# bitmagier/q-learning

Hardware: AMD Instinct MI355X
Metric: env-steps/sec + grad-updates/sec, Breakout 84×84×4, 1/2/4/8 MI355X (higher is better)
Workload: dtype fp32; 1 GPU; C3: 8192 Breakout envs per GPU, replay 1000000 per GPU in HBM (prefilled), Nature-DQN (3 conv + 2 dense) in fp32, B=1024, update every 128 env-steps per GPU (replay ratio 8 samples/env-step), epsilon-greedy acting; envs_per_gpu=8192, batch=1024, replay_capacity=1000000, update_after_actions=128, parallelism=single, rccl_world=1, global_batch_per_update=1024, env_dtype=fp32 physics, u8 frames, qnet_dtype=fp32 (exact-fp32 MFMA v_mfma_f32_16x16x4_f32)

## Files before the change

### q-learning_amd/csrc/qnet32_kernels.h

```cpp
#pragma once
#include <hip/hip_runtime.h>

#include <cstdint>
#include <type_traits>

#include "qlx_internal.h"

namespace qlx {
namespace q32 {

typedef float f32x4 __attribute__((ext_vector_type(4)));

constexpr int BK = 32;
constexpr int kListSlots = 8;
constexpr int kCntStride = 16;

__host__ __device__ constexpr int kmaj_pad(int rows, int r) { return rows + ((r - rows % 64) % 64 + 64) % 64; }
__host__ __device__ constexpr int kmaj_pitch(int rows) {
  return kmaj_pad(rows, 48) < kmaj_pad(rows, 16) ? kmaj_pad(rows, 48) : kmaj_pad(rows, 16);
}
static_assert(kmaj_pitch(32) == 48 && kmaj_pitch(64) == 80 && kmaj_pitch(128) == 144, "KMAJ pitches");

template <int ROWS, bool KMAJ>
struct Opnd {
// ... 409 lines not shown
#pragma unroll
    for (int i = 0; i < N; ++i) {
      const int idx = tid + i * T;
      int r = 0, k = 0;
      if (O::F4 % T == 0 || idx < O::F4) O::coord(idx, r, k);
      vo[i] = lane_off(r, k);
      kk[i] = k;
    }
  }
  __device__ void load(uint32_t soff, int kvalid, Regs& rg) const {
    if (!KMASK || kvalid >= BK) {
#pragma unroll
      for (int i = 0; i < N; ++i)
        if (O::F4 % T == 0 || tid + i * T < O::F4) rg[i] = buf_ld4(rs, vo[i], soff);
    } else {
#pragma unroll
      for (int i = 0; i < N; ++i)
        if (O::F4 % T == 0 || tid + i * T < O::F4) rg[i] = buf_ld4(rs, kk[i] < kvalid ? vo[i] : kOob, soff);
    }
  }
  __device__ void store(float* t, const Regs& rg) const {
#pragma unroll
    for (int i = 0; i < N; ++i) {
      const int idx = tid + i * T;
      if (O::F4 % T == 0 || idx < O::F4) {
        int r, k;
        O::coord(idx, r, k);
        O::put(t, r, k, rg[i]);
      }
    }
  }
};

template <class SA, class SB, uint32_t DA, uint32_t DB, bool KMASK = false>
struct PairStreams {
  SA a;
  SB b;
  int kmax;
  struct Regs {
    typename SA::Regs a;
    typename SB::Regs b;
  };
  __device__ void load(int s, Regs& x) const {
    const int kv = kmax - s * BK;
    a.load((uint32_t)s * DA, kv, x.a);
    b.load((uint32_t)s * DB, kv, x.b);
  }
  __device__ void store(float* as, float* bs, const Regs& x) const {
    a.store(as, x.a);
    b.store(bs, x.b);
  }
};

template <int T, bool PADS = true, int SHIFT = 0, uint32_t MASK = 0xFFFFFFFFu, uint32_t MUL = 1u>
struct TableK4Stream {
  static_assert(T == 256, "table gather stream: four waves");
  using O = Opnd<64, true>;
  static constexpr int N = 2;
  static constexpr uint32_t PAST = SHIFT == 0 && MASK == 0xFFFFFFFFu ? kOob : MASK * MUL;
  using Regs = f32x4[N];
  Rsrc rs;
  uint32_t vo;
  int tid, g, k0;
  const uint32_t* tbl;
  static constexpr int IMG = Opnd<64, true>::FLOATS, PITCH = Opnd<64, true>::PITCH;
  static_assert(PITCH == 80, "table stream: 16 pad columns per k-row");
  __host__ __device__ static int slot(int r) { return PADS ? (r >> 9) * IMG + ((r >> 4) & 31) * PITCH + 64 + (r & 15) : 4 * IMG + r; }
  __device__ void init(const void* base, uint32_t bytes, int tid_, uint32_t row_off) {
    rs = buf_rsrc(base, bytes);
    tid = tid_;
    g = (tid & 63) >> 4;
    k0 = q32_uniform(tid >> 6) * 4;
    vo = row_off;
  }
  __device__ void load(int kbase, Regs& rg) const {
#pragma unroll
    for (int i = 0; i < N; ++i) rg[i] = buf_ld4(rs, vo + ((tbl[slot(kbase + k0 + 16 * i + g)] >> SHIFT) & MASK) * MUL, 0u);
  }
  __device__ void store(float* t, const Regs& rg) const {
#pragma unroll
    for (int i = 0; i < N; ++i) O::put(t, (tid & 15) * 4, k0 + 16 * i + g, rg[i]);
  }
};

template <class P, class = void>
struct ExtraLdsOf : std::integral_constant<size_t, 0> {};
template <class P>
struct ExtraLdsOf<P, std::void_t<decltype(P::EXTRA_LDS)>> : std::integral_constant<size_t, P::EXTRA_LDS> {};

template <class S, class = void>
struct HasPrepare : std::false_type {};
template <class S>
struct HasPrepare<S, std::void_t<decltype(std::declval<S&>().prepare((float*)nullptr, 0))>> : std::true_type {};

template <class P>
constexpr size_t gemm_lds_bytes() {
  return (size_t)KSplitOf<P>::value * 2 *
             (size_t)(Opnd<P::BM, P::A_KMAJ>::FLOATS + Opnd<P::BN, P::B_KMAJ>::FLOATS) * sizeof(float) +
         ExtraLdsOf<P>::value;
}

template <class P, class = void>
struct HasStreams : std::false_type {};
template <class P>
struct HasStreams<P, std::void_t<typename P::Streams>> : std::true_type {};

template <class P>
__device__ __forceinline__ void gemm_body_s(const P& p, int lb, float* lds) {
  constexpr int MF = 16;
  using OA = Opnd<P::BM, P::A_KMAJ>;
  using OB = Opnd<P::BN, P::B_KMAJ>;
  using Acc = f32x4;
  constexpr int TM = P::BM / (P::WM * MF), TN = P::BN / (P::WN * MF);
  static_assert(TM >= 1 && TN >= 1 && TM * P::WM * MF == P::BM && TN * P::WN * MF == P::BN, "tile shape");
  constexpr int G = KSplitOf<P>::value, Q = KSeqOf<P>::value;
  static_assert((G == 1 && Q <= 2) || (Q == 1 && !P::BIAS), "K split: two sequential chains, or wave groups without bias");
  static_assert(G == 1 || TM * TN * 4 * P::WM * P::WN * 64 <= 2 * (OA::FLOATS + OB::FLOATS), "K-split hand-off fits a group's LDS");
  constexpr int T = P::WM * P::WN * 64;
  constexpr int GROUP_LDS = 2 * (OA::FLOATS + OB::FLOATS);
  using St = typename P::Streams;
  using Regs = typename St::Regs;
  const int kg = G > 1 ? __builtin_amdgcn_readfirstlane((int)(threadIdx.x >> 6) / (P::WM * P::WN)) : 0;
  const int tid = threadIdx.x - kg * T, lane = tid & 63;
  const int wave = __builtin_amdgcn_readfirstlane(tid >> 6);
  const int wm = wave % P::WM, wn = wave / P::WM;
  int tm, tn, z;
  p.decode(lb, tm, tn, z);
  const int row0 = tm * P::BM, col0 = tn * P::BN;
  if constexpr (HasActive<P>::value) {
    if (!p.active(z, row0)) return;
  }
  const int ns = p.nslabs(z) / G, s_base = kg * ns;
  const int s_half = Q > 1 ? ns / 2 : -1;
  St st = p.streams(z, row0, col0, tid);
  lds += kg * GROUP_LDS;
  float* As0 = lds;
  float* As1 = lds + OA::FLOATS;
  float* Bs0 = lds + 2 * OA::FLOATS;
  float* Bs1 = Bs0 + OB::FLOATS;
  if constexpr (HasPrepare<St>::value) {
    st.prepare(lds, ns);
    __syncthreads();
  }
  Regs x0, x1;
  Acc acc[TM][TN];
#pragma unroll
  for (int i = 0; i < TM; ++i)
#pragma unroll
    for (int j = 0; j < TN; ++j) acc[i][j] = zero4();
  Acc first[Q > 1 ? TM : 1][Q > 1 ? TN : 1];
  float bsum[TN];
#pragma unroll
  for (int j = 0; j < TN; ++j) bsum[j] = 0.0f;
  const bool do_bias = P::BIAS && tm == 0 && wm == 0;
  auto slab_loop = [&](auto bias_tag) {
    constexpr bool DB = decltype(bias_tag)::value;
    auto compute = [&](int s) {
      const float* a = (s & 1) ? As1 : As0;
      const float* b = (s & 1) ? Bs1 : Bs0;
      if constexpr (Q > 1) {
        if (s == s_half) {
#pragma unroll
          for (int i = 0; i < TM; ++i)
#pragma unroll
            for (int j = 0; j < TN; ++j) {
              first[i][j] = acc[i][j];
// ... 552 lines not shown
    const int m = M;
    st.a.init(dz4, (uint32_t)M * 512u * 4u, tid,
              [row0, m](int r, int k) { return row0 + r < m ? (uint32_t)((row0 + r) * 512 + k) * 4u : kOob; });
    st.b.init(w3, 3136u * 512u * 4u, tid, [col0](int r, int k) { return (uint32_t)((col0 + r) * 512 + k) * 4u; });
    st.kmax = 512;
    return st;
  }
};
using PFc1DgradS = PFc1DgradT<32, 64, 2, 2>;

template <int BM_, int BN_, int WM_, int WN_>
struct PFc1WgradT {
  static constexpr int BM = BM_, BN = BN_, WM = WM_, WN = WN_;
  static constexpr int MINW = 6;
  static constexpr bool A_KMAJ = true, B_KMAJ = true, BIAS = true;
  Grid g;
  const float* a3;
  const float* dz4;
  float* dw3;
  float* db3;
  int B;
  __host__ __device__ void decode(int lb, int& tm, int& tn, int& z) const { g.decode(lb, tm, tn, z); }
  __host__ __device__ int nslabs(int) const { return (B + BK - 1) / BK; }
  __device__ void epi(int, int row, int col, f32x4 v) const {
#pragma unroll
    for (int r = 0; r < 4; ++r)
      if (row + r < 3136) dw3[(size_t)(row + r) * 512 + col] = v[r];
  }
  __device__ void epi_bias(int, int col, float v) const { db3[col] = v; }
  static constexpr int T = WM_ * WN_ * 64;
  using SA = AffineStream<BM_, true, T, true>;
  using SB = AffineStream<BN_, true, T, true>;
  using Streams = PairStreams<SA, SB, BK * 3136u * 4u, BK * 512u * 4u, true>;
  __device__ Streams streams(int, int row0, int col0, int tid) const {
    Streams st;
    st.a.init(a3, (uint32_t)B * 3136u * 4u, tid, [row0](int r, int k) { return (uint32_t)(k * 3136 + row0 + r) * 4u; });
    st.b.init(dz4, (uint32_t)B * 512u * 4u, tid, [col0](int r, int k) { return (uint32_t)(k * 512 + col0 + r) * 4u; });
    st.kmax = B;
    return st;
  }
};
using PFc1WgradS = PFc1WgradT<64, 32, 2, 2>;

__host__ __device__ inline int px3_order(int z) { return z < 5 ? z + 2 : (z == 5 ? 1 : (z == 6 ? 7 : (z == 7 ? 0 : 8))); }
__host__ __device__ inline int px2_order(int z) { return z < 8 ? z + 1 : (z == 8 ? 0 : 9); }

template <int BM_, int BN_, int WM_, int WN_>
struct PConv3DgradPx {
  static constexpr int BM = BM_, BN = BN_, WM = WM_, WN = WN_;
  static constexpr bool LOAD_FENCE = false;
  static constexpr bool A_KMAJ = false, B_KMAJ = false, BIAS = false, RAW_ORDER = true;
  Grid g;
  const float* dz3;
  const float* w2;
  const float* a2;
  float* dz2;
  int B;
  float* pbg = nullptr;
  const uint8_t* bg2 = nullptr;
  int bg2_ld = 0;
  __host__ __device__ void decode(int lb, int& tm, int& tn, int& z) const { g.decode(lb, tm, tn, z); }
  struct Px {
    int ih, iw, kh0, kw0, nkw, ntap;
  };
  struct Pre {
    f32x4 m;
    uint32_t bg;
  };
  __host__ __device__ static Px px(int z) {
    Px q;
    q.ih = px3_order(z / 9);
    q.iw = px3_order(z % 9);
    q.kh0 = q.ih > 6 ? q.ih - 6 : 0;
    q.kw0 = q.iw > 6 ? q.iw - 6 : 0;
    const int kh1 = q.ih < 2 ? q.ih : 2, kw1 = q.iw < 2 ? q.iw : 2;
    q.nkw = kw1 - q.kw0 + 1;
    q.ntap = (kh1 - q.kh0 + 1) * q.nkw;
    return q;
  }
  __host__ __device__ int nslabs(int z) const { return 2 * px(z).ntap; }
  __device__ void epi(int z, int row, int col, f32x4 v) const { epi_post(z, row, col, v, epi_pre(z, row, col)); }
  __device__ Pre epi_pre(int z, int row, int col) const {
    const Px q = px(z);
    Pre pr;
#pragma unroll
    for (int r = 0; r < 4; ++r) pr.m[r] = a2[((size_t)((row + r < B ? row + r : 0) * 9 + q.ih) * 9 + q.iw) * 64 + col];
    pr.bg = pbg ? *reinterpret_cast<const uint32_t*>(bg2 + (size_t)(q.ih * 9 + q.iw) * bg2_ld + row) : 0u;
    return pr;
  }
  __device__ void epi_post(int z, int row, int col, f32x4 v, const Pre& pr) const {
    const Px q = px(z);
    float d[4], e[4];
#pragma unroll
    for (int r = 0; r < 4; ++r) {
      d[r] = row + r < B && pr.m[r] > 0.0f ? v[r] : 0.0f;
      e[r] = ((pr.bg >> (8 * r)) & 0xFFu) != 0u ? d[r] : 0.0f;
      if (row + r < B) dz2[((size_t)((row + r) * 9 + q.ih) * 9 + q.iw) * 64 + col] = d[r];
    }
    if (pbg) {
      const float s = pb_sum16(e);
      if ((row & 15) == 0 && row < B) pbg[((size_t)(row >> 4) * 81 + q.ih * 9 + q.iw) * 64 + col] = s;
    }
  }
  static constexpr int T = WM_ * WN_ * 64;
  struct Streams {
    AffineStream<BM_, false, T> a;
    AffineStream<BN_, false, T> b;
    struct Regs {
      typename AffineStream<BM_, false, T>::Regs a;
      typename AffineStream<BN_, false, T>::Regs b;
    };
    int z0;
    __device__ void load(int s, Regs& x) const {
      const Px q = px(z0);
      const int t = s >> 1, kh = q.kh0 + t / q.nkw, kw = q.kw0 + t % q.nkw, h = (s & 1) * 32;
      a.load((uint32_t)(((q.ih - kh) * 7 + q.iw - kw) * 64 + h) * 4u, 0, x.a);
      b.load((uint32_t)((kh * 3 + kw) * 4096 + h) * 4u, 0, x.b);
    }
    __device__ void store(float* as, float* bs, const Regs& x) const {
      a.store(as, x.a);
      b.store(bs, x.b);
    }
  };
  __device__ Streams streams(int z, int row0, int col0, int tid) const {
    Streams st;
    st.z0 = z;
    const int nb = B;
    st.a.init(dz3, (uint32_t)B * 3136u * 4u, tid,
              [row0, nb](int r, int k) { return row0 + r < nb ? (uint32_t)((row0 + r) * 3136 + k) * 4u : kOob; });
    st.b.init(w2, 9u * 4096u * 4u, tid, [col0](int r, int k) { return (uint32_t)((col0 + r) * 64 + k) * 4u; });
    return st;
  }
};

template <int BM_, int BN_, int WM_, int WN_>
struct PConv2DgradPx {
  static constexpr int BM = BM_, BN = BN_, WM = WM_, WN = WN_;
  static constexpr bool LOAD_FENCE = false;
  static constexpr bool A_KMAJ = false, B_KMAJ = false, BIAS = false, RAW_ORDER = true;
  Grid g;
  const float* dz2;
  const float* w1;
  const float* a1;
  float* dz1;
  int B;
  float* pb = nullptr;
  const uint8_t* need = nullptr;
  int need_ld = 0;
  __host__ __device__ void decode(int lb, int& tm, int& tn, int& z) const { g.decode(lb, tm, tn, z); }
  struct Px {
    int i, j, th0, tw0, ntw, ntap;
  };
  struct Pre {
    f32x4 m;
    uint32_t nb;
  };
  __host__ __device__ static Px px(int z) {
    Px q;
    q.i = px2_order(z / 10);
    q.j = px2_order(z % 10);
    q.th0 = q.i == 9 ? 1 : 0;
    q.tw0 = q.j == 9 ? 1 : 0;
    const int th1 = q.i == 0 ? 0 : 1, tw1 = q.j == 0 ? 0 : 1;
    q.ntw = tw1 - q.tw0 + 1;
    q.ntap = (th1 - q.th0 + 1) * q.ntw;
    return q;
  }
  __host__ __device__ int nslabs(int z) const { return 2 * px(z).ntap; }
  __device__ void epi(int z, int row, int col, f32x4 v) const { epi_post(z, row, col, v, epi_pre(z, row, col)); }
  __device__ Pre epi_pre(int z, int row, int col) const {
    const Px q = px(z);
    const int cls = col >> 5, ih = 2 * q.i + (cls >> 1), iw = 2 * q.j + (cls & 1);
    Pre pr;
#pragma unroll
    for (int r = 0; r < 4; ++r) pr.m[r] = a1[((size_t)((row + r < B ? row + r : 0) * 20 + ih) * 20 + iw) * 32 + (col & 31)];
    pr.nb = need ? *reinterpret_cast<const uint32_t*>(need + (size_t)((ih * 20 + iw) >> 2) * need_ld + row) : ~0u;
    return pr;
  }
  __device__ void epi_post(int z, int row, int col, f32x4 v, const Pre& pr) const {
    const Px q = px(z);
    const int cls = col >> 5, ih = 2 * q.i + (cls >> 1), iw = 2 * q.j + (cls & 1);
    float d[4];
#pragma unroll
    for (int r = 0; r < 4; ++r) {
      d[r] = row + r < B && pr.m[r] > 0.0f ? v[r] : 0.0f;
      if (row + r < B && ((pr.nb >> (8 * r)) & 0xFFu) != 0u) dz1[((size_t)((row + r) * 20 + ih) * 20 + iw) * 32 + (col & 31)] = d[r];
    }
    if (pb) {
      const float s = pb_sum16(d);
      if ((row & 15) == 0 && row < B) pb[((size_t)(row >> 4) * 400 + ih * 20 + iw) * 32 + (col & 31)] = s;
    }
  }
  static constexpr int T = WM_ * WN_ * 64;
  struct Streams {
    AffineStream<BM_, false, T> a;
    AffineStream<BN_, false, T> b;
    Px q;
    struct Regs {
      typename AffineStream<BM_, false, T>::Regs a;
      typename AffineStream<BN_, false, T>::Regs b;
    };
    __device__ void load(int s, Regs& x) const {
      const int t = s >> 1, th = q.th0 + t / q.ntw, tw = q.tw0 + t % q.ntw, h = (s & 1) * 32;
      a.load((uint32_t)(((q.i - th) * 9 + q.j - tw) * 64 + h) * 4u, 0, x.a);
      b.load((uint32_t)((8 * th + 2 * tw) * 2048 + h) * 4u, 0, x.b);
    }
    __device__ void store(float* as, float* bs, const Regs& x) const {
      a.store(as, x.a);
      b.store(bs, x.b);
    }
  };
  __device__ Streams streams(int z, int row0, int col0, int tid) const {
    Streams st;
    st.q = px(z);
    const int nb = B;
    st.a.init(dz2, (uint32_t)B * 5184u * 4u, tid,
              [row0, nb](int r, int k) { return row0 + r < nb ? (uint32_t)((row0 + r) * 5184 + k) * 4u : kOob; });
    st.b.init(w1, 16u * 32u * 64u * 4u, tid, [col0](int r, int k) {
      const int col = col0 + r, cls = col >> 5;
      return (uint32_t)((((cls >> 1) * 4 + (cls & 1)) * 32 + (col & 31)) * 64 + k) * 4u;
    });
    return st;
  }
};

template <int H, int W, int C, int KS, int S, int OH, int OW, int OC, int SC, int BM_ = 64, int BN_ = 64, int WM_ = 2, int WN_ = 2,
          bool TPADS = true, bool CMP = false>
struct PConvWgrad {
  static constexpr int BM = BM_, BN = BN_, WM = WM_, WN = WN_;
  static constexpr bool LOAD_FENCE = false;
  static constexpr bool A_KMAJ = true, B_KMAJ = true, BIAS = true;
  static constexpr int MROWS = KS * KS * C, P = OH * OW, CHUNK = SC;
  Grid g;
  const float* in;
  const float* dz;
  float* slab;
  int B;
  const uint32_t* rows = nullptr;
  __host__ __device__ void decode(int lb, int& tm, int& tn, int& z) const { g.decode(lb, tm, tn, z); }
  __host__ __device__ int rows_in(int z) const {
    const int b0 = z * SC, b1 = b0 + SC < B ? b0 + SC : B;
    return (b1 - b0) * P;
  }
  static_assert(!CMP || (P <= 96 && SC * P <= 4096 && (size_t)SC * H * W * C * 4 <= 0xFFFFFu - 4 * KS * W * C),
                "compacted weight gradient: packed table entries");
  __host__ __device__ int kept_in(int z) const {
    int n = 0;
    for (int bl = 0; bl < SC; ++bl) {
      const int b = z * SC + bl;
      if (b < B) n += __builtin_popcount(rows[(size_t)b * 4]) + __builtin_popcount(rows[(size_t)b * 4 + 1]) +
                      __builtin_popcount(rows[(size_t)b * 4 + 2]);
    }
    return n;
  }
  __host__ __device__ int nslabs(int z) const { return ((CMP ? kept_in(z) : rows_in(z)) + BK - 1) / BK; }
  __device__ void epi(int z, int row, int col, f32x4 v) const {
#pragma unroll
    for (int r = 0; r < 4; ++r) slab[((size_t)z * (MROWS + 1) + row + r) * OC + col] = v[r];
  }
  __device__ void epi_bias(int z, int col, float v) const { slab[((size_t)z * (MROWS + 1) + MROWS) * OC + col] = v; }
  static constexpr int T = WM_ * WN_ * 64;
  static constexpr int KMAX = (SC * P + BK - 1) / BK * BK;
  struct StreamsImpl {
    TableK4Stream<T, TPADS> a;
    AffineStream<BN_, true, T, true> b;
    int z, rows;
    struct Regs {
      typename TableK4Stream<T, TPADS>::Regs a;
      typename AffineStream<BN_, true, T, true>::Regs b;
    };
    __device__ void prepare(float* lds, int ns) {
      uint32_t* t = reinterpret_cast<uint32_t*>(lds);
      for (int r = a.tid; r < ns * BK; r += T) {
        uint32_t o = kOob;
        if (r < rows) {
          const int bl = r / P, pp = r - bl * P, oh = pp / OW, ow = pp - oh * OW;
          o = (uint32_t)((((z * SC + bl) * H + oh * S) * W + ow * S) * C) * 4u;
        }
        t[TableK4Stream<T, TPADS>::slot(r)] = o;
      }
      a.tbl = t;
    }
    __device__ void load(int s, Regs& x) const {
      const int kbase = s * BK;
      a.load(kbase, x.a);
      b.load((uint32_t)kbase * OC * 4u, rows - kbase, x.b);
    }
    __device__ void store(float* as, float* bs, const Regs& x) const {
      a.store(as, x.a);
      b.store(bs, x.b);
    }
  };
  using TA = TableK4Stream<T, TPADS, 0, 0xFFFFFu, 1u>;
  using TB = TableK4Stream<T, TPADS, 20, 0xFFFu, (uint32_t)OC * 4u>;
  struct StreamsCmp {
    TA a;
    TB b;
    int z;
    const uint32_t* rows;
    int B;
    struct Regs {
      typename TA::Regs a;
      typename TB::Regs b;
    };
    __device__ void prepare(float* lds, int ns) {
      uint32_t* t = reinterpret_cast<uint32_t*>(lds);
      int run = 0;
      for (int bl = 0; bl < SC; ++bl) {
        const int b = z * SC + bl;
        if (b >= B) break;
        const uint32_t w0 = rows[(size_t)b * 4], w1 = rows[(size_t)b * 4 + 1], w2 = rows[(size_t)b * 4 + 2];
        for (int pp = a.tid; pp < P; pp += T) {
          const uint32_t w = pp < 32 ? w0 : (pp < 64 ? w1 : w2), bit = 1u << (pp & 31);
          if (w & bit) {
            const int below = (pp >= 32 ? __builtin_popcount(w0) : 0) + (pp >= 64 ? __builtin_popcount(w1) : 0) +
                              __builtin_popcount(w & (bit - 1u));
            const int oh = pp / OW, ow = pp - oh * OW;
            const uint32_t ao = (uint32_t)(((bl * H + oh * S) * W + ow * S) * C) * 4u;
            t[TA::slot(run + below)] = ao | ((uint32_t)(bl * P + pp) << 20);
          }
        }
        run += __builtin_popcount(w0) + __builtin_popcount(w1) + __builtin_popcount(w2);
      }
      for (int r = run + a.tid; r < ns * BK; r += T) t[TA::slot(r)] = 0xFFFFFFFFu;
      a.tbl = t;
      b.tbl = t;
    }
    __device__ void load(int s, Regs& x) const {
      a.load(s * BK, x.a);
      b.load(s * BK, x.b);
    }
    __device__ void store(float* as, float* bs, const Regs& x) const {
      a.store(as, x.a);
      b.store(bs, x.b);
    }
  };
  static_assert(BM_ == 64 && WM_ * WN_ == 4, "weight gradient: the table stream stages 64-row tiles on four waves");
  using Streams = std::conditional_t<CMP, StreamsCmp, StreamsImpl>;
  static_assert(!TPADS || KMAX <= 4 * 32 * 16, "weight-gradient chunk: the offset table lives in the four images' pads");
  static_assert(!TPADS || BN_ == 64, "weight-gradient tiles with the table in the pads need BN = 64");
  static constexpr size_t EXTRA_LDS = !TPADS ? (size_t)KMAX * 4 : 0;
  __device__ Streams streams(int z, int row0, int col0, int tid) const {
    Streams st;
    st.z = z;
    const int m = row0 + (tid & 15) * 4, tap = m / C, c = m - tap * C, kh = tap / KS, kw = tap - kh * KS;
    if constexpr (CMP) {
      st.rows = rows;
      st.B = B;
      const int nb = B - z * SC < SC ? B - z * SC : SC;
      st.a.init(in + (size_t)z * SC * H * W * C, (uint32_t)nb * H * W * C * 4u, tid, (uint32_t)((kh * W + kw) * C + c) * 4u);
      st.b.init(dz + (size_t)z * SC * P * OC, (uint32_t)nb * P * OC * 4u, tid, (uint32_t)(col0 + (tid & 15) * 4) * 4u);
    } else {
      st.rows = rows_in(z);
      st.a.init(in, (uint32_t)B * H * W * C * 4u, tid, (uint32_t)((kh * W + kw) * C + c) * 4u);
      st.b.init(dz + (size_t)z * SC * P * OC, (uint32_t)st.rows * OC * 4u, tid,
                [col0](int r, int k) { return (uint32_t)(k * OC + col0 + r) * 4u; });
    }
    return st;
  }
};

constexpr int kSC1 = QLX_F32_WGRAD_CHUNK_CONV1, kSC2 = QLX_F32_WGRAD_CHUNK_CONV2, kSC3 = QLX_F32_WGRAD_CHUNK_CONV3;
using PConv3Wgrad = PConvWgrad<9, 9, 64, 3, 1, 7, 7, 64, kSC3, 64, 64, 1, 4, false, true>;
using PConv3WgradD = PConvWgrad<9, 9, 64, 3, 1, 7, 7, 64, kSC3, 64, 64, 1, 4, false>;
static_assert(kSC3 == 16, "conv3 weight-gradient chunks are the fc1 backward's 16-row fragments (pbg)");
using PConv2Wgrad = PConvWgrad<20, 20, 32, 4, 2, 9, 9, 64, kSC2, 64, 64, 1, 4, true, true>;
using PConv2WgradD = PConvWgrad<20, 20, 32, 4, 2, 9, 9, 64, kSC2, 64, 64, 1, 4>;
static_assert(kSC2 == 16, "conv2 weight-gradient chunks are the conv3 backward's 16-row fragments (pbg)");
using PConv3DgradP = PConv3DgradPx<64, 64, 2, 2>;
using PConv2DgradP = PConv2DgradPx<64, 64, 2, 2>;

template <bool DQ>
struct SideFc2T {
  static constexpr int BLOCKS = 33;
  __host__ __device__ int blocks() const { return BLOCKS; }
  static constexpr int HB = 512;
  static constexpr size_t LDS = (size_t)HB * 20 * sizeof(float);
  const float* a4;
  const uint8_t* act;
  const float* gs;
  const float* hs;
  int B;
  float* dw4;
  float* db4;
  float* loss;
  const float* dq = nullptr;
  __device__ void run(int t, float* lds) const {
    float* as = lds;
    float* ds = lds + HB * 16;
    const int tid = threadIdx.x, lane = tid & 63, g = lane >> 4, n = lane & 15;
    f32x4 acc = zero4();
    for (int b0 = 0; b0 < B; b0 += HB) {
      __syncthreads();
      if (t < 32) {
// ... 74 lines not shown
  const uint8_t* hi = (slot & 1) ? f.p[3] : f.p[2];
  return (slot & 2) ? hi : lo;
}

__device__ __forceinline__ void c1_prefetch(const C1Ptrs& f, uint4 (&pf)[7]) {
#pragma unroll
  for (int j = 0; j < 7; ++j) {
    const int q = threadIdx.x + 256 * j;
    const bool ok = q < kC1Chunks;
    const int qq = ok ? q : 0, slot = qq / 441, pos = qq - slot * 441;
    pf[j] = ldg_frame(ok ? c1_slot(f, slot) : nullptr, pos);
  }
}
__device__ __forceinline__ void c1_put(uint32_t* dst, int q, const uint4& v) {
  const int slot = q / 441, pos = q - slot * 441, bx = pos / 21, by = pos - bx * 21;
  uint32_t* d = dst + slot * kC1SlotDw + 4 * bx * 21 + by;
  d[0] = v.x;
  d[21] = v.y;
  d[42] = v.z;
  d[63] = v.w;
}
__device__ __forceinline__ void c1_stage(uint32_t* dst, const uint4 (&pf)[7]) {
#pragma unroll
  for (int j = 0; j < 7; ++j) {
    const int q = threadIdx.x + 256 * j;
    if (q < kC1Chunks) c1_put(dst, q, pf[j]);
  }
}
__device__ __forceinline__ float ubyte(uint32_t w, int i) { return (float)((w >> (8 * i)) & 0xFFu); }

struct C1Lists {
  int* rl2;
  int* rl3;
  int cap2, cap3;
  unsigned long long* cnt;
  unsigned long long* cnt_next;
  float* xbg;
  uint32_t* steps;
  uint8_t* need;
  int need_ld;
  uint32_t* rows2;
  uint8_t* bg2;
  uint32_t* rows3;
  uint8_t* bg3;
};
constexpr int kC1RmDw = 24;

__device__ __forceinline__ int c1_opaque_tid() {
  int t = threadIdx.x;
  asm volatile("" : "+v"(t));
  return t;
}
__device__ __forceinline__ void c1_mark(uint32_t* rm, const uint4 (&pf)[7]) {
  const int t = c1_opaque_tid();
#pragma unroll
  for (int j = 0; j < 7; ++j) {
    const int q = t + 256 * j;
    if (q < kC1Chunks && (pf[j].x | pf[j].y | pf[j].z | pf[j].w) != 0u) {
      const int pos = q % 441, bx = pos / 21, by = pos - bx * 21;
      atomicOr(&rm[bx], 1u << by);
    }
  }
}

__device__ __forceinline__ void c1_steps(const uint32_t* rm, uint32_t* out, uint8_t* need, int need_ld, int b, int lane) {
  bool nd[2];
#pragma unroll
  for (int h = 0; h < 2; ++h) {
    const int s = lane + 64 * h;
    const bool valid = s < 100;
    const int ss = valid ? s : 0, oh = ss / 5, t = ss - 5 * oh;
    nd[h] = valid && ((((rm[oh] | rm[oh + 1]) >> (4 * t)) & 0x1Fu) != 0u);
    if (need && valid) need[(size_t)s * need_ld + b] = nd[h] ? 1 : 0;
  }
  const unsigned long long m0 = __builtin_amdgcn_ballot_w64(nd[0]), m1 = __builtin_amdgcn_ballot_w64(nd[1]);
  if (lane < 4) {
    const unsigned long long m = lane < 2 ? m0 : m1;
    out[lane] = (uint32_t)(m >> (32 * (lane & 1)));
  }
}
__device__ __forceinline__ bool c1_step_set(unsigned long long lo, unsigned long long hi, int st) {
  return ((st < 64 ? lo >> st : hi >> (st - 64)) & 1ull) != 0ull;
}

__device__ __forceinline__ void c1_flags(const uint32_t* rm, unsigned long long* cl, int wave, const C1Lists& L, int b) {
  const int tid = c1_opaque_tid();
  const int R = wave < 2 ? 81 : 49, p = wave < 2 ? tid : tid - 128;
  const bool valid = p < R;
  const int pp = valid ? p : 0;
  bool nonbg;
  if (wave < 2) {
    const int i = pp / 9, j = pp - 9 * i;
    uint32_t mm = 0;
#pragma unroll
    for (int r = 0; r < 5; ++r) mm |= rm[2 * i + r];
    nonbg = ((mm >> (2 * j)) & 0x1Fu) != 0u;
  } else {
    const int i = pp / 7, j = pp - 7 * i;
    uint32_t mm = 0;
#pragma unroll
    for (int r = 0; r < 9; ++r) mm |= rm[2 * i + r];
    nonbg = ((mm >> (2 * j)) & 0x1FFu) != 0u;
  }
  const unsigned long long bn = __builtin_amdgcn_ballot_w64(valid && nonbg), bb = __builtin_amdgcn_ballot_w64(valid && !nonbg);
  if ((tid & 63) == 0) {
    cl[0] = bn;
    cl[1] = bb;
  }
  if (wave < 2 && L.rows2) {
    const int lane = tid & 63;
    if (lane < 2 && (wave == 0 || lane == 0)) L.rows2[(size_t)b * 4 + 2 * wave + lane] = (uint32_t)(bn >> (32 * lane));
    if (wave == 1 && lane == 1) L.rows2[(size_t)b * 4 + 3] = 0u;
    if (valid) L.bg2[(size_t)p * L.need_ld + b] = nonbg ? 0 : 1;
  }
  if (wave == 2 && L.rows3) {
    const int lane = tid & 63;
    if (lane < 4) L.rows3[(size_t)b * 4 + lane] = lane < 2 ? (uint32_t)(bn >> (32 * lane)) : 0u;
    if (valid) L.bg3[(size_t)p * L.need_ld + b] = nonbg ? 0 : 1;
  }
}
__device__ __forceinline__ void c1_lists_flush(const unsigned long long* cl, int nit, int b0, int G, const C1Lists& L, int wave,
                                               int tid, unsigned long long* xch) {
  const int lane = tid & 63, R = wave < 2 ? 81 : 49, p = wave < 2 ? tid : tid - 128;
  int* rl = wave < 2 ? L.rl2 : L.rl3;
  auto wave_tot = [&](int wv) {
    unsigned long long t = 0;
    for (int it = 0; it < nit; ++it)
      t += ((unsigned long long)__builtin_popcountll(cl[(it * 3 + wv) * 2]) << 32) |
           (unsigned long long)__builtin_popcountll(cl[(it * 3 + wv) * 2 + 1]);
    return t;
  };
  unsigned long long old = 0;
  const int slot = blockIdx.x % kListSlots, cap = wave < 2 ? L.cap2 : L.cap3;
  rl += slot * cap;
  if ((wave == 0 || wave == 2) && lane == 0) {
    const unsigned long long tot = wave == 0 ? wave_tot(0) + wave_tot(1) : wave_tot(2);
    old = __hip_atomic_fetch_add(L.cnt + (slot * 2 + (wave < 2 ? 0 : 1)) * kCntStride, tot, __ATOMIC_RELAXED, __HIP_MEMORY_SCOPE_AGENT);
    if (wave == 0) *xch = old;
  }
  __syncthreads();
  if (wave == 1) old = *xch + wave_tot(0);
  if (wave >= 3) return;
  old = __shfl(old, 0);
  int on = (int)(old >> 32), og = (int)(uint32_t)old;
  const unsigned long long below = (1ull << lane) - 1ull;
  for (int it = 0; it < nit; ++it) {
    const unsigned long long bn = cl[(it * 3 + wave) * 2], bb = cl[(it * 3 + wave) * 2 + 1];
    const int e = (b0 + it * G) * R + p;
    int tap = 0;
    if (wave == 2) {
      const unsigned long long g0 = cl[(it * 3) * 2 + 1], g1 = cl[(it * 3 + 1) * 2 + 1];
      const int i = p / 7, j = p - 7 * (p / 7);
#pragma unroll
      for (int t = 0; t < 9; ++t) {
        const int q = (i + t / 3) * 9 + j + t % 3;
        tap |= (int)(((q < 64 ? g0 >> q : g1 >> (q - 64)) & 1ull) << t);
      }
    }
    if ((bn >> lane) & 1ull) rl[on + __builtin_popcountll(bn & below)] = e | (tap << 20);
    else if ((bb >> lane) & 1ull) rl[cap - 1 - (og + __builtin_popcountll(bb & below))] = e;
    on += __builtin_popcountll(bn);
    og += __builtin_popcountll(bb);
  }
}

__device__ __forceinline__ void c1_fwd_sample(const uint32_t* fr, const uint32_t (&ob2)[7], int nt, int rp, int g, int col,
                                              const float (&wf)[64], float bias, int skip, float* a1, int b) {
  {
    uint32_t dn[16];
    auto tile_dwords = [&](int j, uint32_t (&d)[16]) {
      const uint32_t base = (ob2[j >> 1] >> (16 * (j & 1))) & 0xFFFFu;
#pragma unroll
      for (int kq = 0; kq < 16; ++kq) d[kq] = fr[base + (kq >> 1) * 21 + (kq & 1)];
    };
    tile_dwords(0, dn);
#pragma unroll
    for (int j = 0; j < 13; ++j)
      if (j < nt) {
        uint32_t d[16];
#pragma unroll
        for (int kq = 0; kq < 16; ++kq) d[kq] = dn[kq];
        bool nz[16];
#pragma unroll
        for (int kq = 0; kq < 16; ++kq) nz[kq] = (__builtin_amdgcn_ballot_w64(d[kq] != 0u) != 0) | (skip == 0);
        if (j + 1 < nt) tile_dwords(j + 1, dn);
        f32x4 acc = zero4();
#pragma unroll
        for (int kq = 0; kq < 16; ++kq)
          if (nz[kq])
#pragma unroll
            for (int kw = 0; kw < 4; ++kw) acc = __builtin_amdgcn_mfma_f32_16x16x4f32(ubyte(d[kq], kw), wf[kq * 4 + kw], acc, 0, 0, 0);
        const int t = rp + 2 * j, r0 = (4 * (t / 5) + g) * 20 + 4 * (t % 5);
#pragma unroll
        for (int i = 0; i < 4; ++i) a1[((size_t)b * 400 + r0 + i) * 32 + col] = relu(acc[i] + bias);
      }
  }
}

constexpr int kC1OneMinW = 4;
template <int ROLE, bool ONE = false>
__global__ __launch_bounds__(256, ONE ? kC1OneMinW : 2) void k_conv1_fwd32(const uint8_t* const* table, int B, const float* w0,
                                                                           const float* b0, float* a1, int skip, const C1Lists L) {
  extern __shared__ __attribute__((aligned(16))) uint32_t c1w[];
  uint32_t* rm = c1w + (ONE ? 1 : 2) * 4 * kC1SlotDw;
  unsigned long long* cl = reinterpret_cast<unsigned long long*>(rm + 3 * kC1RmDw);
  const bool lists = L.rl2 != nullptr;
  const bool marks = lists || L.rows2 != nullptr || L.rows3 != nullptr;
  const int tid = threadIdx.x, lane = tid & 63;
  const int wave = __builtin_amdgcn_readfirstlane(tid >> 6);
  if (marks) {
    if (blockIdx.x == 0 && tid < 2 * kListSlots) L.cnt_next[tid * kCntStride] = 0ull;
    if (blockIdx.x == 0 && tid < 32) L.xbg[tid] = relu(0.0f + b0[tid]);
    if (tid < 3 * kC1RmDw) rm[tid] = 0u;
    __syncthreads();
  }
  const int ct = wave & 1, rp = wave >> 1;
  const int col = ct * 16 + (lane & 15), g = lane >> 4;
  float wf[64];
#pragma unroll
  for (int kk = 0; kk < 64; ++kk) wf[kk] = w0[(kk * 4 + g) * 32 + col];
  const float bias = b0[col];
  uint32_t ob2[7];
#pragma unroll
  for (int j = 0; j < 7; ++j) ob2[j] = 0;
#pragma unroll
  for (int j = 0; j < 13; ++j) {
    const int t = rp + 2 * j < 25 ? rp + 2 * j : 0, l = lane & 15;
    const int oh = 4 * (t / 5) + (l >> 2), ow = 4 * (t % 5) + (l & 3);
    ob2[j >> 1] |= (uint32_t)(g * kC1SlotDw + 4 * oh * 21 + ow) << (16 * (j & 1));
  }
  const int nt = rp == 0 ? 13 : 12;
  int b = blockIdx.x;
  if (b >= B) return;
  if constexpr (ONE) {
    {
      uint4 pf[7];
      c1_prefetch(c1_ptrs(table, b), pf);
      c1_stage(c1w, pf);
      if (marks) c1_mark(rm, pf);
    }
    __syncthreads();
    c1_fwd_sample(c1w, ob2, nt, rp, g, col, wf, bias, skip, a1, b);
    if (marks) {
      if (wave < 3) c1_flags(rm, cl + wave * 2, wave, L, b);
      else if (L.steps) c1_steps(rm, L.steps + (size_t)b * 4, L.need, L.need_ld, b, lane);
      if (lists) {
        __syncthreads();
        c1_lists_flush(cl, 1, blockIdx.x, gridDim.x, L, wave, tid, cl + 6);
      }
    }
    return;
  }
  uint4 pf[7];
  c1_prefetch(c1_ptrs(table, b), pf);
  C1Ptrs nxt = c1_ptrs(table, b + (int)gridDim.x < B ? b + (int)gridDim.x : b);
  c1_stage(c1w, pf);
  if (marks) c1_mark(rm, pf);
  __syncthreads();
  for (int it = 0; b < B; b += gridDim.x, ++it) {
    const uint32_t* fr = c1w + (it & 1) * (4 * kC1SlotDw);
    const int nb = b + gridDim.x;
    if (nb < B) {
      c1_prefetch(nxt, pf);
      nxt = c1_ptrs(table, nb + (int)gridDim.x < B ? nb + (int)gridDim.x : nb);
    }
    if (marks && wave == 3 && tid - 192 < kC1RmDw) rm[((it + 2) % 3) * kC1RmDw + tid - 192] = 0u;
    c1_fwd_sample(fr, ob2, nt, rp, g, col, wf, bias, skip, a1, b);
    if (marks && wave < 3) c1_flags(rm + (it % 3) * kC1RmDw, cl + it * 6 + wave * 2, wave, L, b);
    if (marks && wave == 3 && L.steps) c1_steps(rm + (it % 3) * kC1RmDw, L.steps + (size_t)b * 4, L.need, L.need_ld, b, lane);
    if (nb < B) {
      c1_stage(c1w + ((it + 1) & 1) * (4 * kC1SlotDw), pf);
      if (marks) c1_mark(rm + ((it + 1) % 3) * kC1RmDw, pf);
    }
    __syncthreads();
  }
  if (lists) {
    const int nit = (B - (int)blockIdx.x + (int)gridDim.x - 1) / (int)gridDim.x;
    c1_lists_flush(cl, nit, blockIdx.x, gridDim.x, L, wave, tid, cl + nit * 6);
  }
}

constexpr int kC1DzChunks = 400 * 32 / 4;
constexpr int kC1WgSlotDw = 1768;
constexpr int kC1WgradThreads = 512;
constexpr int kC1WgradPf = (kC1Chunks + kC1DzChunks + kC1WgradThreads - 1) / kC1WgradThreads;
constexpr size_t kC1WgradLds = (size_t)4 * kC1WgSlotDw * 4 + (size_t)400 * 32 * 4;
__host__ __device__ constexpr int c1_wgrad_blocks(int nz) { return nz; }
__global__ __launch_bounds__(kC1WgradThreads, 2) void k_conv1_wgrad32(const uint8_t* const* table, const float* dz1, int B, int nz,
                                                                       float* slab, int skip, const uint32_t* steps,
                                                                       const float* pb) {
  extern __shared__ __attribute__((aligned(16))) uint32_t c1w[];
  float* dzs = reinterpret_cast<float*>(c1w + 4 * kC1WgSlotDw);
  const int tid = threadIdx.x, lane = tid & 63;
  const int wave = __builtin_amdgcn_readfirstlane(tid >> 6);
  const int z = blockIdx.x, hh = wave >> 2, wq = wave & 3;
  const int g = lane >> 4, l15 = lane & 15;
  const int b0 = z * QLX_F32_WGRAD_CHUNK_CONV1;
  const int nb = min(QLX_F32_WGRAD_CHUNK_CONV1, B - b0);
  const int ao = (l15 & 3) * kC1WgSlotDw + (2 * wq + (l15 >> 3)) * 21 + ((l15 >> 2) & 1);
  const int bo = hh * 16 + l15;

  const int boc = tid & 31, bjb = tid >> 5;
  float bt = 0.0f;
  {
    const int NR = ((B + 15) >> 4) * 400, R = (NR + nz - 1) / nz, i0 = z * R, i1 = min(NR, i0 + R);
    for (int i = i0 + bjb; i < i1; i += 64) {
      float v[4];
#pragma unroll
      for (int u = 0; u < 4; ++u) v[u] = i + 16 * u < i1 ? pb[(size_t)(i + 16 * u) * 32 + boc] : 0.0f;
#pragma unroll
      for (int u = 0; u < 4; ++u)
        if (i + 16 * u < i1) bt = __fadd_rn(bt, v[u]);
    }
  }
  uint4 pf[kC1WgradPf];
  auto prefetch = [&](int b, uint4 (&pf)[kC1WgradPf]) {
    const C1Ptrs f = c1_ptrs(table, b);
    const uint64_t zp = (uint64_t)(gbyte*)q32_zero4;
    const uint64_t dzb = (uint64_t)(dz1 + (size_t)b * 400 * 32);
    unsigned long long lo = ~0ull, hi = ~0ull;
    if (steps) {
      cu32* sp = (cu32*)(steps + (size_t)b * 4);
      lo = (unsigned long long)sp[0] | ((unsigned long long)sp[1] << 32);
      hi = (unsigned long long)sp[2] | ((unsigned long long)sp[3] << 32);
    }
#pragma unroll
    for (int j = 0; j < kC1WgradPf; ++j) {
      const int q = tid + kC1WgradThreads * j;
      const bool isf = q < kC1Chunks, isd = !isf && q < kC1Chunks + kC1DzChunks;
      const int qf = isf ? q : 0, slot = qf / 441, pos = qf - slot * 441;
      const int e = isd ? q - kC1Chunks : 0;
      const uint64_t fp = (uint64_t)c1_slot(f, slot);
      const uint64_t fa = fp ? fp + (uint64_t)(pos * 16) : zp;
      const uint64_t da = c1_step_set(lo, hi, e >> 5) ? dzb + (uint64_t)e * 16 : zp;
      const u32x4v v = *(gu4*)(isf ? fa : (isd ? da : zp));
      pf[j] = uint4{v.x, v.y, v.z, v.w};
    }
  };
  auto stage = [&](const uint4 (&pf)[kC1WgradPf]) {
#pragma unroll
    for (int j = 0; j < kC1WgradPf; ++j) {
      const int q = tid + kC1WgradThreads * j;
      if (q < kC1Chunks) {
        const int slot = q / 441, pos = q - slot * 441, bx = pos / 21, by = pos - bx * 21;
        uint32_t* d = c1w + slot * kC1WgSlotDw + 4 * bx * 21 + by;
        d[0] = pf[j].x;
        d[21] = pf[j].y;
        d[42] = pf[j].z;
        d[63] = pf[j].w;
      } else if (q < kC1Chunks + kC1DzChunks) {
        const int e = q - kC1Chunks, r = e >> 3, part = e & 7;
        *reinterpret_cast<uint4*>(dzs + (part >> 2) * 6400 + r * 16 + (part & 3) * 4) = pf[j];
      }
    }
  };
  f32x4 acc[4];
#pragma unroll
  for (int t = 0; t < 4; ++t) acc[t] = zero4();
  prefetch(b0, pf);
#pragma unroll
  for (int bl = 0; bl < QLX_F32_WGRAD_CHUNK_CONV1; ++bl) {
    if (bl >= nb) break;
    __syncthreads();
    stage(pf);
    __syncthreads();
    if (bl + 1 < nb) prefetch(b0 + bl + 1, pf);
    constexpr int GS = 5, NG = 100 / GS;
    static_assert(NG % 2 == 0 && NG * GS == 100, "conv1 weight gradient: operand groups");
    float bA[GS], bB[GS];
    uint32_t xA[GS], xB[GS];
    auto rd = [&](int grp, float (&bv)[GS], uint32_t (&px)[GS]) {
#pragma unroll
      for (int j = 0; j < GS; ++j) {
        const int r = 4 * (grp * GS + j) + g, oh = r / 20, ow = r - oh * 20;
        bv[j] = dzs[hh * 6400 + r * 16 + l15];
        px[j] = c1w[ao + 84 * oh + ow];
      }
    };
    auto run = [&](const float (&bv)[GS], const uint32_t (&px)[GS]) {
      bool nz[GS];
#pragma unroll
      for (int j = 0; j < GS; ++j) nz[j] = (__builtin_amdgcn_ballot_w64(px[j] != 0u) != 0) | (skip == 0);
#pragma unroll
      for (int j = 0; j < GS; ++j) {
        if (nz[j])
#pragma unroll
          for (int t = 0; t < 4; ++t) acc[t] = __builtin_amdgcn_mfma_f32_16x16x4f32(ubyte(px[j], t), bv[j], acc[t], 0, 0, 0);
      }
    };
    rd(0, bA, xA);
    for (int grp = 0; grp < NG; grp += 2) {
      rd(grp + 1, bB, xB);
      run(bA, xA);
      if (grp + 2 < NG) rd(grp + 2, bA, xA);
      run(bB, xB);
    }
  }
  float* out = slab + (size_t)z * 257 * 32;
#pragma unroll
  for (int t = 0; t < 4; ++t)
#pragma unroll
    for (int i = 0; i < 4; ++i) {
      const int rho = 4 * g + i, kh = 2 * wq + (rho >> 3), kw = 4 * ((rho >> 2) & 1) + t, c = rho & 3;
      out[(size_t)((kh * 8 + kw) * 4 + c) * 32 + bo] = acc[t][i];
    }
  __syncthreads();
  dzs[bjb * 32 + boc] = bt;
  __syncthreads();
  if (tid < 32) {
    float sb = 0.0f;
#pragma unroll
    for (int j = 0; j < 16; ++j) sb = __fadd_rn(sb, dzs[j * 32 + tid]);
    out[256 * 32 + tid] = sb;
  }
}

#endif

}
}
```

Before: 321,700 env-steps/s.

## Skip dead conv1 tiles, use 32-bit epilogue offsets, wave-broadcast row masks

Several independent micro-optimisations land together across the Q-network kernels. The conv2/conv3 backward epilogues switch to 32-bit byte offsets in place of 64-bit index maths. The compacted weight-gradient row counting and prepare load the row words once per wave and broadcast them with readlane instead of issuing repeated scalar loads. Conv1 forward builds a per-lane mask of live 4x4 tiles from the frame marks, skips the MFMAs for all-zero tiles and writes relu(bias) directly. Conv1 wgrad precomputes LDS offsets and fully unrolls its group loop, which may raise register pressure.

```diff
diff --git a/q-learning_amd/csrc/qnet32_kernels.h b/q-learning_amd/csrc/qnet32_kernels.h
--- a/q-learning_amd/csrc/qnet32_kernels.h
+++ b/q-learning_amd/csrc/qnet32_kernels.h
@@ -515,6 +515,13 @@
     for (int i = 0; i < N; ++i) O::put(t, (tid & 15) * 4, k0 + 16 * i + g, rg[i]);
   }
 };
+
+__host__ __device__ inline float ld_off(const float* base, uint32_t off) {
+  return *reinterpret_cast<const float*>(reinterpret_cast<const char*>(base) + off);
+}
+__host__ __device__ inline void st_off(float* base, uint32_t off, float v) {
+  *reinterpret_cast<float*>(reinterpret_cast<char*>(base) + off) = v;
+}
 
 template <class P, class = void>
 struct ExtraLdsOf : std::integral_constant<size_t, 0> {};
@@ -1233,20 +1240,22 @@
   __device__ void epi(int z, int row, int col, f32x4 v) const { epi_post(z, row, col, v, epi_pre(z, row, col)); }
   __device__ Pre epi_pre(int z, int row, int col) const {
     const Px q = px(z);
+    const uint32_t po = (uint32_t)((q.ih * 9 + q.iw) * 64 + col) * 4u;
     Pre pr;
 #pragma unroll
-    for (int r = 0; r < 4; ++r) pr.m[r] = a2[((size_t)((row + r < B ? row + r : 0) * 9 + q.ih) * 9 + q.iw) * 64 + col];
+    for (int r = 0; r < 4; ++r) pr.m[r] = ld_off(a2, (uint32_t)(row + r < B ? row + r : 0) * 20736u + po);
     pr.bg = pbg ? *reinterpret_cast<const uint32_t*>(bg2 + (size_t)(q.ih * 9 + q.iw) * bg2_ld + row) : 0u;
     return pr;
   }
   __device__ void epi_post(int z, int row, int col, f32x4 v, const Pre& pr) const {
     const Px q = px(z);
+    const uint32_t po = (uint32_t)((q.ih * 9 + q.iw) * 64 + col) * 4u;
     float d[4], e[4];
 #pragma unroll
     for (int r = 0; r < 4; ++r) {
       d[r] = row + r < B && pr.m[r] > 0.0f ? v[r] : 0.0f;
       e[r] = ((pr.bg >> (8 * r)) & 0xFFu) != 0u ? d[r] : 0.0f;
-      if (row + r < B) dz2[((size_t)((row + r) * 9 + q.ih) * 9 + q.iw) * 64 + col] = d[r];
+      if (row + r < B) st_off(dz2, (uint32_t)(row + r) * 20736u + po, d[r]);
     }
     if (pbg) {
       const float s = pb_sum16(e);
@@ -1322,20 +1331,22 @@
   __device__ Pre epi_pre(int z, int row, int col) const {
     const Px q = px(z);
     const int cls = col >> 5, ih = 2 * q.i + (cls >> 1), iw = 2 * q.j + (cls & 1);
+    const uint32_t po = (uint32_t)((ih * 20 + iw) * 32 + (col & 31)) * 4u;
     Pre pr;
 #pragma unroll
-    for (int r = 0; r < 4; ++r) pr.m[r] = a1[((size_t)((row + r < B ? row + r : 0) * 20 + ih) * 20 + iw) * 32 + (col & 31)];
+    for (int r = 0; r < 4; ++r) pr.m[r] = ld_off(a1, (uint32_t)(row + r < B ? row + r : 0) * 51200u + po);
     pr.nb = need ? *reinterpret_cast<const uint32_t*>(need + (size_t)((ih * 20 + iw) >> 2) * need_ld + row) : ~0u;
     return pr;
   }
   __device__ void epi_post(int z, int row, int col, f32x4 v, const Pre& pr) const {
     const Px q = px(z);
     const int cls = col >> 5, ih = 2 * q.i + (cls >> 1), iw = 2 * q.j + (cls & 1);
+    const uint32_t po = (uint32_t)((ih * 20 + iw) * 32 + (col & 31)) * 4u;
     float d[4];
 #pragma unroll
     for (int r = 0; r < 4; ++r) {
       d[r] = row + r < B && pr.m[r] > 0.0f ? v[r] : 0.0f;
-      if (row + r < B && ((pr.nb >> (8 * r)) & 0xFFu) != 0u) dz1[((size_t)((row + r) * 20 + ih) * 20 + iw) * 32 + (col & 31)] = d[r];
+      if (row + r < B && ((pr.nb >> (8 * r)) & 0xFFu) != 0u) st_off(dz1, (uint32_t)(row + r) * 51200u + po, d[r]);
     }
     if (pb) {
       const float s = pb_sum16(d);
@@ -1397,6 +1408,16 @@
                 "compacted weight gradient: packed table entries");
   __host__ __device__ int kept_in(int z) const {
     int n = 0;
+#if defined(__HIP_DEVICE_COMPILE__) && !defined(QLX_Q32_POLICIES_ONLY)
+    if constexpr (CMP) {
+      static_assert(SC * 4 == 64, "compacted weight gradient: a chunk's row words are one wave's lanes");
+      const int wl = threadIdx.x & 63;
+      const uint32_t wv = z * SC + (wl >> 2) < B && (wl & 3) != 3 ? rows[(size_t)z * SC * 4 + wl] : 0u;
+      for (int l = 0; l < 64; ++l)
+        if ((l & 3) != 3) n += __builtin_popcount(__builtin_amdgcn_readlane(wv, l));
+      return n;
+    }
+#endif
     for (int bl = 0; bl < SC; ++bl) {
       const int b = z * SC + bl;
       if (b < B) n += __builtin_popcount(rows[(size_t)b * 4]) + __builtin_popcount(rows[(size_t)b * 4 + 1]) +
@@ -1457,10 +1478,20 @@
     __device__ void prepare(float* lds, int ns) {
       uint32_t* t = reinterpret_cast<uint32_t*>(lds);
       int run = 0;
+#ifndef QLX_Q32_POLICIES_ONLY
+      static_assert(SC * 4 == 64, "compacted weight gradient: a chunk's row words are one wave's lanes");
+      const int wl = a.tid & 63;
+      const uint32_t wv = z * SC + (wl >> 2) < B ? rows[(size_t)z * SC * 4 + wl] : 0u;
+#endif
       for (int bl = 0; bl < SC; ++bl) {
+#ifdef QLX_Q32_POLICIES_ONLY
         const int b = z * SC + bl;
-        if (b >= B) break;
-        const uint32_t w0 = rows[(size_t)b * 4], w1 = rows[(size_t)b * 4 + 1], w2 = rows[(size_t)b * 4 + 2];
+        const uint32_t w0 = b < B ? rows[(size_t)b * 4] : 0u, w1 = b < B ? rows[(size_t)b * 4 + 1] : 0u,
+                       w2 = b < B ? rows[(size_t)b * 4 + 2] : 0u;
+#else
+        const uint32_t w0 = __builtin_amdgcn_readlane(wv, 4 * bl), w1 = __builtin_amdgcn_readlane(wv, 4 * bl + 1),
+                       w2 = __builtin_amdgcn_readlane(wv, 4 * bl + 2);
+#endif
         for (int pp = a.tid; pp < P; pp += T) {
           const uint32_t w = pp < 32 ? w0 : (pp < 64 ? w1 : w2), bit = 1u << (pp & 31);
           if (w & bit) {
@@ -1701,7 +1732,13 @@
 __device__ __forceinline__ bool c1_step_set(unsigned long long lo, unsigned long long hi, int st) {
   return ((st < 64 ? lo >> st : hi >> (st - 64)) & 1ull) != 0ull;
 }
-
+__device__ __forceinline__ uint32_t c1_tiles(const uint32_t* rm, int lane) {
+  const int t = lane < 25 ? lane : 0, bx = 4 * (t / 5), by = 4 * (t % 5);
+  uint32_t mm = 0;
+#pragma unroll
+  for (int r = 0; r < 5; ++r) mm |= rm[bx + r];
+  return (uint32_t)__builtin_amdgcn_ballot_w64(lane < 25 && ((mm >> by) & 0x1Fu) != 0u);
+}
 __device__ __forceinline__ void c1_flags(const uint32_t* rm, unsigned long long* cl, int wave, const C1Lists& L, int b) {
   const int tid = c1_opaque_tid();
   const int R = wave < 2 ? 81 : 49, p = wave < 2 ? tid : tid - 128;
@@ -1783,36 +1820,47 @@
   }
 }
 
-__device__ __forceinline__ void c1_fwd_sample(const uint32_t* fr, const uint32_t (&ob2)[7], int nt, int rp, int g, int col,
-                                              const float (&wf)[64], float bias, int skip, float* a1, int b) {
+__device__ __forceinline__ void c1_fwd_sample(const uint32_t* fr, uint32_t lb, int nt, int rp, int g, int col,
+                                              const float (&wf)[64], float bias, int skip, uint32_t live, float* a1, int b) {
   {
-    uint32_t dn[16];
+    const unsigned long long every = skip == 0 ? ~0ull : 0ull;
+    auto tile_live = [&](int j) { return ((live >> (rp + 2 * j)) & 1u) != 0u; };
     auto tile_dwords = [&](int j, uint32_t (&d)[16]) {
-      const uint32_t base = (ob2[j >> 1] >> (16 * (j & 1))) & 0xFFFFu;
+      const int t = rp + 2 * j;
+      const uint32_t base = lb + (uint32_t)((t / 5) * (16 * 21) + (t % 5) * 4);
 #pragma unroll
       for (int kq = 0; kq < 16; ++kq) d[kq] = fr[base + (kq >> 1) * 21 + (kq & 1)];
     };
-    tile_dwords(0, dn);
-#pragma unroll
-    for (int j = 0; j < 13; ++j)
-      if (j < nt) {
-        uint32_t d[16];
-#pragma unroll
-        for (int kq = 0; kq < 16; ++kq) d[kq] = dn[kq];
+    const uint32_t so = (uint32_t)(g * 20 * 32 + col);
+    const float zb = relu(0.0f + bias);
+    auto tile = [&](int j, const uint32_t (&d)[16], uint32_t (&dn)[16]) {
+      const bool lv = tile_live(j), nx = j + 1 < nt && tile_live(j + 1);
+      const int t = rp + 2 * j;
+      float* at = a1 + ((size_t)b * 400 + 80 * (t / 5) + 4 * (t % 5)) * 32;
+      if (lv) {
         bool nz[16];
 #pragma unroll
-        for (int kq = 0; kq < 16; ++kq) nz[kq] = (__builtin_amdgcn_ballot_w64(d[kq] != 0u) != 0) | (skip == 0);
-        if (j + 1 < nt) tile_dwords(j + 1, dn);
+        for (int kq = 0; kq < 16; ++kq) nz[kq] = (__builtin_amdgcn_ballot_w64(d[kq] != 0u) | every) != 0ull;
+        if (nx) tile_dwords(j + 1, dn);
         f32x4 acc = zero4();
 #pragma unroll
         for (int kq = 0; kq < 16; ++kq)
           if (nz[kq])
 #pragma unroll
             for (int kw = 0; kw < 4; ++kw) acc = __builtin_amdgcn_mfma_f32_16x16x4f32(ubyte(d[kq], kw), wf[kq * 4 + kw], acc, 0, 0, 0);
-        const int t = rp + 2 * j, r0 = (4 * (t / 5) + g) * 20 + 4 * (t % 5);
-#pragma unroll
-        for (int i = 0; i < 4; ++i) a1[((size_t)b * 400 + r0 + i) * 32 + col] = relu(acc[i] + bias);
-      }
+#pragma unroll
+        for (int i = 0; i < 4; ++i) at[so + 32u * i] = relu(acc[i] + bias);
+      } else {
+        if (nx) tile_dwords(j + 1, dn);
+#pragma unroll
+        for (int i = 0; i < 4; ++i) at[so + 32u * i] = zb;
+      }
+    };
+    uint32_t dd[14][16];
+    if (tile_live(0)) tile_dwords(0, dd[0]);
+#pragma unroll
+    for (int j = 0; j < 13; ++j)
+      if (j < nt) tile(j, dd[j], dd[j + 1]);
   }
 }
 
@@ -1839,15 +1887,7 @@
 #pragma unroll
   for (int kk = 0; kk < 64; ++kk) wf[kk] = w0[(kk * 4 + g) * 32 + col];
   const float bias = b0[col];
-  uint32_t ob2[7];
-#pragma unroll
-  for (int j = 0; j < 7; ++j) ob2[j] = 0;
-#pragma unroll
-  for (int j = 0; j < 13; ++j) {
-    const int t = rp + 2 * j < 25 ? rp + 2 * j : 0, l = lane & 15;
-    const int oh = 4 * (t / 5) + (l >> 2), ow = 4 * (t % 5) + (l & 3);
-    ob2[j >> 1] |= (uint32_t)(g * kC1SlotDw + 4 * oh * 21 + ow) << (16 * (j & 1));
-  }
+  const uint32_t lb = (uint32_t)(g * kC1SlotDw + 4 * ((lane & 15) >> 2) * 21 + (lane & 3));
   const int nt = rp == 0 ? 13 : 12;
   int b = blockIdx.x;
   if (b >= B) return;
@@ -1859,7 +1899,7 @@
       if (marks) c1_mark(rm, pf);
     }
     __syncthreads();
-    c1_fwd_sample(c1w, ob2, nt, rp, g, col, wf, bias, skip, a1, b);
+    c1_fwd_sample(c1w, lb, nt, rp, g, col, wf, bias, skip, marks && skip != 0 ? c1_tiles(rm, lane) : ~0u, a1, b);
     if (marks) {
       if (wave < 3) c1_flags(rm, cl + wave * 2, wave, L, b);
       else if (L.steps) c1_steps(rm, L.steps + (size_t)b * 4, L.need, L.need_ld, b, lane);
@@ -1884,7 +1924,8 @@
       nxt = c1_ptrs(table, nb + (int)gridDim.x < B ? nb + (int)gridDim.x : nb);
     }
     if (marks && wave == 3 && tid - 192 < kC1RmDw) rm[((it + 2) % 3) * kC1RmDw + tid - 192] = 0u;
-    c1_fwd_sample(fr, ob2, nt, rp, g, col, wf, bias, skip, a1, b);
+    c1_fwd_sample(fr, lb, nt, rp, g, col, wf, bias, skip, marks && skip != 0 ? c1_tiles(rm + (it % 3) * kC1RmDw, lane) : ~0u, a1,
+                  b);
     if (marks && wave < 3) c1_flags(rm + (it % 3) * kC1RmDw, cl + it * 6 + wave * 2, wave, L, b);
     if (marks && wave == 3 && L.steps) c1_steps(rm + (it % 3) * kC1RmDw, L.steps + (size_t)b * 4, L.need, L.need_ld, b, lane);
     if (nb < B) {
@@ -1918,6 +1959,8 @@
   const int nb = min(QLX_F32_WGRAD_CHUNK_CONV1, B - b0);
   const int ao = (l15 & 3) * kC1WgSlotDw + (2 * wq + (l15 >> 3)) * 21 + ((l15 >> 2) & 1);
   const int bo = hh * 16 + l15;
+  const int pxo = ao + g, dzo = hh * 6400 + g * 16 + l15;
+  const unsigned long long every = skip == 0 ? ~0ull : 0ull;
 
   const int boc = tid & 31, bjb = tid >> 5;
   float bt = 0.0f;
@@ -1986,20 +2029,20 @@
     if (bl + 1 < nb) prefetch(b0 + bl + 1, pf);
     constexpr int GS = 5, NG = 100 / GS;
     static_assert(NG % 2 == 0 && NG * GS == 100, "conv1 weight gradient: operand groups");
+    static_assert(GS == 5, "conv1 weight gradient: a group is one output row");
     float bA[GS], bB[GS];
     uint32_t xA[GS], xB[GS];
     auto rd = [&](int grp, float (&bv)[GS], uint32_t (&px)[GS]) {
 #pragma unroll
       for (int j = 0; j < GS; ++j) {
-        const int r = 4 * (grp * GS + j) + g, oh = r / 20, ow = r - oh * 20;
-        bv[j] = dzs[hh * 6400 + r * 16 + l15];
-        px[j] = c1w[ao + 84 * oh + ow];
+        bv[j] = dzs[dzo + grp * 320 + j * 64];
+        px[j] = c1w[pxo + grp * 84 + j * 4];
       }
     };
     auto run = [&](const float (&bv)[GS], const uint32_t (&px)[GS]) {
       bool nz[GS];
 #pragma unroll
-      for (int j = 0; j < GS; ++j) nz[j] = (__builtin_amdgcn_ballot_w64(px[j] != 0u) != 0) | (skip == 0);
+      for (int j = 0; j < GS; ++j) nz[j] = (__builtin_amdgcn_ballot_w64(px[j] != 0u) | every) != 0ull;
 #pragma unroll
       for (int j = 0; j < GS; ++j) {
         if (nz[j])
@@ -2008,6 +2051,7 @@
       }
     };
     rd(0, bA, xA);
+#pragma unroll
     for (int grp = 0; grp < NG; grp += 2) {
       rd(grp + 1, bB, xB);
       run(bA, xA);
```

Result: faster. 331,900 env-steps/s (median of 6 runs) (+3.2%).
